# Rudrabha/Wav2Lip

Measured on NVIDIA H100. Metric: 96x96 face-crops/sec (B=128, T=5, mel 80x16), higher is better.
Workload: dtype f16

## Files before the change

wav2lip_b200/csrc/convt_fused.cuh:

```cuda
#pragma once

#include "conv_igemm.cuh"

namespace w2l {

constexpr int kCtThreads = 384;
constexpr int kCtBN = 64;
constexpr int kCtPW = 9, kCtPH = 17;
constexpr int kCtMaxStages = 6;

struct alignas(64) ConvTParams {
    CUtensorMap tmA;
    CUtensorMap tmB;
    CUtensorMap tmO[4];
    int tiles_x, tiles_y, N;
    int kc;
    int stages;
    int patch_bytes, patch_stride;
    int act;
    float cscale[64], cshift[64];
};

template <int G, int BK, bool kBF16>
__device__ __forceinline__ void convt_consumer(const ConvTParams& p, uint32_t smem_base, uint32_t stg, uint32_t bar_base) {
    constexpr int BN = kCtBN;
    constexpr int kRowBytes = BK * 2;
    constexpr int kSlab = BN * BK * 2;
    constexpr uint32_t kSboA = kCtPW * kRowBytes;
    constexpr uint32_t kSboB = 8 * kRowBytes;
    constexpr uint32_t kRowB = BN * 2;
    const int kc = p.kc;
    const int stages = p.stages;
    const uint32_t stage_bytes = p.patch_stride + 9u * kSlab;
    auto full_bar = [&](int s) { return bar_base + 8u * s; };
    auto empty_bar = [&](int s) { return bar_base + 8u * (kCtMaxStages + s); };
    const int lane = threadIdx.x & 31;
    const int q = (threadIdx.x >> 5) & 3;
    const bool leader = (q == 0 && lane == 0);
    const uint32_t bar_id = 1 + G;
    const int tiles_per_img = p.tiles_x * p.tiles_y;
    const int total_units = tiles_per_img * p.N;
    float acc[2][64];
    int stage = 0;
    uint32_t phase = 0;
    for (int unit = blockIdx.x; unit < total_units; unit += gridDim.x) {
        const int n = unit / tiles_per_img;
        const int r = unit - n * tiles_per_img;
        const int ty = r / p.tiles_x, tx = r - ty * p.tiles_x;
        int prev = -1;
        for (int c = 0; c < kc; ++c) {
            mbar_wait(full_bar(stage), phase);
            const uint32_t patch = smem_base + stage * stage_bytes;
            const uint32_t wslab = patch + p.patch_stride;
            wg_fence();
#pragma unroll
            for (int k = 0; k < BK / 16; ++k) {
                const uint32_t on = (c | k) != 0 ? 1u : 0u;
#pragma unroll
                for (int h = 0; h < 2; ++h) {
                    const uint32_t a0 = patch + h * 8 * kSboA + 32u * k;
                    auto ad = [&](uint32_t rows) { return wg_desc(a0 + rows * kRowBytes, 16, kSboA, kRowBytes); };
                    auto bd = [&](int slab) { return wg_desc(wslab + slab * kSlab + 32u * k, 16, kSboB, kRowBytes); };
                    if constexpr (G == 0) {
                        wgmma_m64k16<128, kBF16>(acc[h], ad(0), bd(0), on, 0);
                        wgmma_m64k16<64, kBF16>(acc[h] + 32, ad(1), bd(4), 1u, 0);
                        wgmma_m64k16<64, kBF16>(acc[h] + 32, ad(kCtPW), bd(5), 1u, 0);
                        wgmma_m64k16<64, kBF16>(acc[h] + 32, ad(kCtPW + 1), bd(6), 1u, 0);
                    } else {
                        wgmma_m64k16<128, kBF16>(acc[h], ad(0), bd(2), on, 0);
                        wgmma_m64k16<64, kBF16>(acc[h], ad(1), bd(7), 1u, 0);
                        wgmma_m64k16<64, kBF16>(acc[h] + 32, ad(kCtPW), bd(8), 1u, 0);
                    }
                }
            }
            wg_commit();
            wg_wait<1>();
            if (prev >= 0 && lane == 0) mbar_arrive(empty_bar(prev));
            prev = stage;
            if (++stage == stages) { stage = 0; phase ^= 1u; }
        }
        wg_wait<0>();
        wg_fence_regs<64>(acc[0]);
        wg_fence_regs<64>(acc[1]);
        if (prev >= 0 && lane == 0) mbar_arrive(empty_bar(prev));
#pragma unroll
        for (int lp = 0; lp < 2; ++lp) {
            const int ph = G == 0 ? 3 * lp : 1 + lp;
            if (leader) asm volatile("cp.async.bulk.wait_group.read 0;" ::: "memory");
            named_bar_sync(bar_id, 128);
#pragma unroll
            for (int j = 0; j < 8; ++j) {
                const int cc = 8 * j + 2 * (lane & 3);
                const float sc0 = p.cscale[cc], sc1 = p.cscale[cc + 1], sh0 = p.cshift[cc], sh1 = p.cshift[cc + 1];
#pragma unroll
                for (int h = 0; h < 2; ++h) {
#pragma unroll
                    for (int r8 = 0; r8 < 2; ++r8) {
                        const int row = 64 * h + 16 * q + (lane >> 2) + 8 * r8;
                        float f0 = fmaf(acc[h][4 * (8 * lp + j) + 2 * r8], sc0, sh0);
                        float f1 = fmaf(acc[h][4 * (8 * lp + j) + 2 * r8 + 1], sc1, sh1);
                        if (p.act == ACT_RELU) {
                            f0 = fmaxf(f0, 0.0f);
                            f1 = fmaxf(f1, 0.0f);
                        } else if (p.act == ACT_LRELU) {
                            f0 = f0 > 0.0f ? f0 : 0.01f * f0;
                            f1 = f1 > 0.0f ? f1 : 0.01f * f1;
                        }
                        uint32_t a = stg + row * kRowB + cc * 2;
                        a ^= ((a >> 7) & 7u) << 4;
                        asm volatile("st.shared.b32 [%0], %1;" ::"r"(a), "r"(pack2<kBF16>(f0, f1)) : "memory");
                    }
                }
            }
            asm volatile("fence.proxy.async.shared::cta;" ::: "memory");
            named_bar_sync(bar_id, 128);
            if (leader) {
                asm volatile("cp.async.bulk.tensor.4d.global.shared::cta.bulk_group [%0, {%2, %3, %4, %5}], [%1];"
                             ::"l"(reinterpret_cast<uint64_t>(&p.tmO[ph])), "r"(stg), "r"(0), "r"(tx * 8), "r"(ty * 16), "r"(n)
                             : "memory");
                asm volatile("cp.async.bulk.commit_group;" ::: "memory");
            }
        }
    }
    if (leader) asm volatile("cp.async.bulk.wait_group 0;" ::: "memory");
}

template <int BK, bool kBF16>
__global__ void __launch_bounds__(kCtThreads, 1) convt_fused_kernel(const __grid_constant__ ConvTParams p) {
    pdl_launch_dependents();
    constexpr uint32_t kStgBytes = kTileM * kCtBN * 2;
    constexpr int kSlab = kCtBN * BK * 2;

    extern __shared__ uint8_t smem_raw[];
    const uint32_t smem_base = (smem_u32(smem_raw) + 1023u) & ~1023u;
    const int kc = p.kc;
    const int stages = p.stages;
    const uint32_t stage_bytes = p.patch_stride + 9u * kSlab;
    const uint32_t stg_base = smem_base + stages * stage_bytes;
    const uint32_t bar_base = stg_base + 2u * kStgBytes;
    auto full_bar = [&](int s) { return bar_base + 8u * s; };
    auto empty_bar = [&](int s) { return bar_base + 8u * (kCtMaxStages + s); };

    const int warp = threadIdx.x >> 5;
    const int lane = threadIdx.x & 31;

    if (warp == 0 && lane == 0) {
        tma_prefetch_desc(&p.tmA);
        tma_prefetch_desc(&p.tmB);
#pragma unroll
        for (int i = 0; i < 4; ++i) tma_prefetch_desc(&p.tmO[i]);
    }
    if (warp == 1 && lane == 0) {
        for (int s = 0; s < stages; ++s) {
            mbar_init(full_bar(s), 1);
            mbar_init(empty_bar(s), 8);
        }
        fence_barrier_init();
    }
    __syncthreads();
    pdl_wait();

    const int tiles_per_img = p.tiles_x * p.tiles_y;
    const int total_units = tiles_per_img * p.N;

    if (warp < 4) {
        setmaxnreg_dec<kProducerRegs>();
        if (warp == 0 && lane == 0) {
            int stage = 0;
            uint32_t phase = 0;
            for (int unit = blockIdx.x; unit < total_units; unit += gridDim.x) {
                const int n = unit / tiles_per_img;
                const int r = unit - n * tiles_per_img;
                const int ty = r / p.tiles_x, tx = r - ty * p.tiles_x;
                for (int c = 0; c < kc; ++c) {
                    mbar_wait(empty_bar(stage), phase ^ 1u);
                    const uint32_t a_dst = smem_base + stage * stage_bytes;
                    mbar_arrive_expect_tx(full_bar(stage), static_cast<uint32_t>(p.patch_bytes) + 9u * kSlab);
                    tma_load_4d(a_dst, &p.tmA, full_bar(stage), c * BK, tx * 8, ty * 16, n);
                    tma_load_3d(a_dst + p.patch_stride, &p.tmB, full_bar(stage), c * BK, 0, 0);
                    if (++stage == stages) { stage = 0; phase ^= 1u; }
                }
            }
        }
    } else {
        setmaxnreg_inc<kConsumerRegs>();
        if (warp >= 8)
            convt_consumer<1, BK, kBF16>(p, smem_base, stg_base + kStgBytes, bar_base);
        else
            convt_consumer<0, BK, kBF16>(p, smem_base, stg_base, bar_base);
    }
}

}
```

wav2lip_b200/csrc/host_ops.cuh:

```cuda
#pragma once

static int pick_bk(int cin_pad) { return (cin_pad % 64 == 0) ? 64 : (cin_pad % 32 == 0) ? 32 : 16; }
static int round_up(int a, int b) { return (a + b - 1) / b * b; }
constexpr int kCmMinSteps = 18;
constexpr int kCmMinCtaSteps = 48;
constexpr double kCmFillMargin = 0.06;

static void pick_box(int W, int H, int N, int sx, int sy, int* bw, int* bh, int* bn, int pixels = kTileM) {
    double best = 1e30;
    int b_w = 1, b_h = 1, b_n = 1;
    for (int w = 1; w <= std::min(W, pixels); ++w) {
        if (w * sx > 256) break;
        for (int h = 1; h <= std::min(H, pixels / w); ++h) {
            if (h * sy > 256) break;
            int n = std::min(pixels / (w * h), std::max(N, 1));
            if (n < 1) continue;
            if (n > 256) n = 256;
            const double tiles = (double)((W + w - 1) / w) * ((H + h - 1) / h) * ((N + n - 1) / n);
            const double cost = tiles - 1e-6 * w - 1e-9 * h;
            if (cost < best) { best = cost; b_w = w; b_h = h; b_n = n; }
        }
    }
    *bw = b_w; *bh = b_h; *bn = b_n;
}
// ... 233 lines not shown
    p.bw = bw; p.bh = bh; p.bn = bn;
    p.sx = a.sx; p.sy = a.sy;
    p.ntaps = w.ntaps; p.kc_per_tap = w.cin_pad / BK;
    p.stage_tx_bytes = (unsigned)(op.MT * bw * bh * bn * BK * 2 + BN * BK * 2);
    fill_epi(&p.ep, a);
    p.tma_epi = 0;
    if (ctx->use_tma_epi && !ctx->x2 && !a.head && !a.out.f32) {
        EncodeTiledFn enc = get_encode_fn();
        const int EW = BN < 64 ? BN : 64;
        const CUtensorMapDataType dt = ctx->bf16 ? CU_TENSOR_MAP_DATA_TYPE_BFLOAT16 : CU_TENSOR_MAP_DATA_TYPE_FLOAT16;
        const CUtensorMapSwizzle esw = EW == 64 ? CU_TENSOR_MAP_SWIZZLE_128B : EW == 32 ? CU_TENSOR_MAP_SWIZZLE_64B : CU_TENSOR_MAP_SWIZZLE_32B;
        cuuint64_t dims[4] = {(cuuint64_t)std::min(a.cout, a.out.C), (cuuint64_t)a.Wl, (cuuint64_t)a.Hl, (cuuint64_t)a.in.N};
        cuuint32_t box[4] = {(cuuint32_t)EW, (cuuint32_t)bw, (cuuint32_t)bh, (cuuint32_t)bn};
        cuuint32_t es[4] = {1, 1, 1, 1};
        cuuint64_t os[3] = {(cuuint64_t)p.ep.out_sx * 2, (cuuint64_t)p.ep.out_sy * 2, (cuuint64_t)p.ep.out_sn * 2};
        CUresult r = enc(&p.tmO, dt, 4, p.ep.out, dims, os, box, es, CU_TENSOR_MAP_INTERLEAVE_NONE, esw,
                         CU_TENSOR_MAP_L2_PROMOTION_L2_128B, CU_TENSOR_MAP_FLOAT_OOB_FILL_NONE);
        if (r != CUDA_SUCCESS) return fail(W2L_ECUDA, "%s: cuTensorMapEncodeTiled(out) failed with %d", a.name.c_str(), (int)r);
        if (a.res) {
            cuuint64_t rs[3] = {(cuuint64_t)p.ep.res_sx * 2, (cuuint64_t)p.ep.res_sy * 2, (cuuint64_t)p.ep.res_sn * 2};
            r = enc(&p.tmR, dt, 4, const_cast<void*>(p.ep.res), dims, rs, box, es, CU_TENSOR_MAP_INTERLEAVE_NONE, esw,
                    CU_TENSOR_MAP_L2_PROMOTION_L2_128B, CU_TENSOR_MAP_FLOAT_OOB_FILL_NONE);
            if (r != CUDA_SUCCESS) return fail(W2L_ECUDA, "%s: cuTensorMapEncodeTiled(res) failed with %d", a.name.c_str(), (int)r);
        } else {
            p.tmR = p.tmO;
        }
        p.tma_epi = 1;
        p.epi_box_bytes = (unsigned)(bw * bh * bn * EW * 2);
    }
    if (w.ntaps > kMaxTaps) return fail(W2L_EINVAL, "%s: too many taps", a.name.c_str());
    if (a.cout > a.out.C && !p.tma_epi && !a.head) return fail(W2L_ESTATE, "%s: %d computed channels for a %d-channel destination need the TMA-store epilogue", a.name.c_str(), a.cout, a.out.C);
    if (ctx->x2) {
        if (a.in.lo_off <= 0 || w.nslabs != 2 * w.ntaps) return fail(W2L_ESTATE, "%s: split-operand mode needs hi/lo planes", a.name.c_str());
        int k = 0;
        for (int t = 0; t < w.ntaps; ++t)
            for (int v = 0; v < 3; ++v, ++k) {
                p.dx[k] = w.dx[t]; p.dy[k] = w.dy[t];
                p.a_lo[k] = (v == 1) ? 1 : 0;
                p.b_slab[k] = (unsigned char)((v == 2) ? w.ntaps + t : t);
            }
        p.ntaps = 3 * w.ntaps;
        p.a_lo_off = a.in.lo_off;
    } else {
        for (int t = 0; t < w.ntaps; ++t) { p.dx[t] = w.dx[t]; p.dy[t] = w.dy[t]; p.a_lo[t] = 0; p.b_slab[t] = (unsigned char)t; }
    }
    const int total = ((m_tiles + op.MT - 1) / op.MT) * p.n_tiles;
    op.grid = std::min(total, ctx->num_sms);
    op.fold = w.fold; op.m_tiles = m_tiles; op.n_tiles = p.n_tiles;
    op.flops = 2.0 * a.macs_per_pixel * (double)a.Wl * a.Hl * a.in.N;
    pl->ops.push_back(op);
    return W2L_OK;
}

static int make_convt_fused_op(w2l_ctx* ctx, Plan* pl, const Layer& L, const LayerW& lw, const Act& in, const Act& out, int act = ACT_RELU) {
    EncodeTiledFn enc = get_encode_fn();
    if (!enc) return fail(W2L_ENODEV, "cuTensorMapEncodeTiled is not available");
    const PackedW& w = lw.ph.back();
    Op op;
    op.type = OP_CONV;
    op.name = L.name + " [fused 4-phase]";
    op.ctf = true;
    const int BK = 32;
    if (w.cin_pad % BK != 0) return fail(W2L_EINVAL, "%s: fused convT needs cin %% 32 == 0", L.name.c_str());
    op.BK = BK; op.BN = kCtBN;
    ConvTParams& t = op.tp;
    memset(&t, 0, sizeof(t));
    CKR(encode_act_map(ctx, &t.tmA, in, BK, kCtPW, kCtPH, 1, 1, 1, L.name.c_str()));
    {
        const CUtensorMapDataType dt = ctx->bf16 ? CU_TENSOR_MAP_DATA_TYPE_BFLOAT16 : CU_TENSOR_MAP_DATA_TYPE_FLOAT16;
        const CUtensorMapSwizzle sw = CU_TENSOR_MAP_SWIZZLE_64B;
        cuuint64_t dims[3] = {(cuuint64_t)w.cin_pad, (cuuint64_t)w.cout_pad, 9};
        cuuint64_t strides[2] = {(cuuint64_t)w.cin_pad * 2, (cuuint64_t)w.cin_pad * w.cout_pad * 2};
        cuuint32_t box[3] = {(cuuint32_t)BK, (cuuint32_t)kCtBN, 9};
        cuuint32_t es[3] = {1, 1, 1};
        CUresult r = enc(&t.tmB, dt, 3, w.w, dims, strides, box, es, CU_TENSOR_MAP_INTERLEAVE_NONE, sw,
                         CU_TENSOR_MAP_L2_PROMOTION_L2_256B, CU_TENSOR_MAP_FLOAT_OOB_FILL_NONE);
        if (r != CUDA_SUCCESS) return fail(W2L_ECUDA, "%s: cuTensorMapEncodeTiled(B9) failed with %d", L.name.c_str(), (int)r);
        for (int py = 0; py < 2; ++py)
            for (int px = 0; px < 2; ++px) {
                uint16_t* base = out.base + ((long long)py * out.W + px) * out.Cs + out.c_off;
                cuuint64_t od[4] = {(cuuint64_t)kCtBN, (cuuint64_t)in.W, (cuuint64_t)in.H, (cuuint64_t)in.N};
                cuuint64_t os[3] = {(cuuint64_t)2 * out.Cs * 2, (cuuint64_t)2 * out.W * out.Cs * 2, (cuuint64_t)out.H * out.W * out.Cs * 2};
                cuuint32_t ob[4] = {(cuuint32_t)kCtBN, 8, 16, 1};
                cuuint32_t oe[4] = {1, 1, 1, 1};
                CUresult r2 = enc(&t.tmO[py * 2 + px], dt, 4, base, od, os, ob, oe, CU_TENSOR_MAP_INTERLEAVE_NONE,
                                  CU_TENSOR_MAP_SWIZZLE_128B, CU_TENSOR_MAP_L2_PROMOTION_L2_128B, CU_TENSOR_MAP_FLOAT_OOB_FILL_NONE);
                if (r2 != CUDA_SUCCESS) return fail(W2L_ECUDA, "%s: cuTensorMapEncodeTiled(out phase) failed with %d", L.name.c_str(), (int)r2);
            }
    }
    t.tiles_x = (in.W + 7) / 8; t.tiles_y = (in.H + 15) / 16; t.N = in.N;
    t.kc = w.cin_pad / BK;
    t.patch_bytes = kCtPW * kCtPH * BK * 2;
    t.patch_stride = (t.patch_bytes + 1023) / 1024 * 1024;
    const int stage_bytes = t.patch_stride + 9 * kCtBN * BK * 2;
    const int fixed = 2 * kTileM * kCtBN * 2 + kSmemExtra;
    t.stages = std::min(kCtMaxStages, (kCtSmemMax - fixed) / stage_bytes);
    if (t.stages < 2) return fail(W2L_EINVAL, "%s: fused convT does not fit shared memory", L.name.c_str());
    op.dyn_smem = t.stages * stage_bytes + fixed;
    t.act = act;
    CK(cudaDeviceSynchronize());
    CK(cudaMemcpy(t.cscale, lw.scale, kCtBN * 4, cudaMemcpyDeviceToHost));
    CK(cudaMemcpy(t.cshift, lw.shift, kCtBN * 4, cudaMemcpyDeviceToHost));
    const long long units = (long long)t.tiles_x * t.tiles_y * in.N;
    op.grid = (int)std::min<long long>(units, ctx->num_sms);
    op.m_tiles = (int)units; op.n_tiles = 1;
    op.flops = 2.0 * (double)L.cin * L.cout * 9 * (double)in.W * in.H * in.N;
    pl->ops.push_back(op);
    return W2L_OK;
}

static int emit_block(w2l_ctx* ctx, Plan* pl, const NetW& nw, int li, const Layer& L, const Act& in, const Act& out,
                      const Act* res, bool head = false, int head_B = 1, int head_T = 1, int act_override = -1) {
    const LayerW& lw = nw.layers[li];
    ConvArgs a;
    a.in = in; a.out = out; a.res = res;
    a.scale = lw.scale; a.shift = lw.shift;
    a.act = (L.kind == W2L_BLOCK_CONV_LRELU) ? ACT_LRELU : (L.kind == W2L_BLOCK_CONV_PLAIN ? ACT_NONE : ACT_RELU);
    if (act_override >= 0) a.act = act_override;
    a.cout = L.cout;
    a.head = head; a.head_w = nw.head_w; a.head_b = nw.head_b; a.head_B = head_B; a.head_T = head_T;
    if (L.kind != W2L_BLOCK_CONVT_BN_RELU) {
        a.name = L.name;
        a.w = &lw.ph[0];
        a.sx = lw.ph[0].fold ? 1 : L.sw; a.sy = L.sh;
        a.Hl = out.H; a.Wl = out.W;
        a.macs_per_pixel = (double)L.cin * L.cout * L.kh * L.kw;
        return make_conv_op(ctx, pl, a);
    }
    if (lw.gemm_convT) {
        Act o = out;
        o.H = 1; o.W = 1; o.Cs = out.Cs * out.H * out.W; o.C = L.cout * L.kh * L.kw;
        if (out.c_off != 0 || out.C != out.Cs) return fail(W2L_EINVAL, "%s: gemm convT needs a dense output", L.name.c_str());
        a.name = L.name;
        a.out = o;
        a.w = &lw.ph[0];
        a.Hl = 1; a.Wl = 1;
        a.cout = L.cout * L.kh * L.kw;
        a.macs_per_pixel = (double)L.cin * L.cout * L.kh * L.kw;
        return make_conv_op(ctx, pl, a);
    }
    if (lw.has_all_taps && ctx->use_ctfused && lw.ph.back().cin_pad % 32 == 0 && in.W >= 8 && in.H >= 8 && !res &&
        out.H == 2 * in.H && out.W == 2 * in.W &&
        (double)in.W * in.H / ((double)((in.W + 7) / 8) * ((in.H + 15) / 16) * kTileM) >= 0.6 && !out.f32)
        return make_convt_fused_op(ctx, pl, L, lw, in, out, a.act);
    const size_t nph = lw.ph.size() - (lw.has_all_taps ? 1 : 0);
    for (size_t i = 0; i < nph; ++i) {
        const PackedW& w = lw.ph[i];
        ConvArgs b = a;
        b.name = L.name + ".ph" + std::to_string(w.py) + std::to_string(w.px);
        b.w = &w;
        b.osy = L.sh; b.osx = L.sw; b.phy = w.py; b.phx = w.px;
        b.Hl = (out.H - w.py + L.sh - 1) / L.sh;
        b.Wl = (out.W - w.px + L.sw - 1) / L.sw;
        b.macs_per_pixel = (double)L.cin * L.cout * w.ntaps;
        CKR(make_conv_op(ctx, pl, b));
    }
    return W2L_OK;
}

static void conv_out_dims(const Layer& L, int H, int W, int* Ho, int* Wo) {
    if (L.kind == W2L_BLOCK_CONVT_BN_RELU) {
        *Ho = (H - 1) * L.sh - 2 * L.ph + L.kh + L.out_pad;
        *Wo = (W - 1) * L.sw - 2 * L.pw + L.kw + L.out_pad;
    } else {
        *Ho = (H + 2 * L.ph - L.kh) / L.sh + 1;
        *Wo = (W + 2 * L.pw - L.kw) / L.sw + 1;
    }
}
```

wav2lip_b200/csrc/host_weights.cuh:

```cuda
#pragma once

struct TensorRef { const float* p; int64_t n; };
typedef std::map<std::string, TensorRef> TensorMap;

static int need(const TensorMap& tm, const std::string& name, int64_t numel, const float** out) {
    auto it = tm.find(name);
    if (it == tm.end()) return fail(W2L_EINVAL, "missing tensor '%s'", name.c_str());
    if (it->second.n != numel) return fail(W2L_EINVAL, "tensor '%s' has %lld elements, expected %lld", name.c_str(), (long long)it->second.n, (long long)numel);
    *out = it->second.p;
    return W2L_OK;
}

static int pack_taps(w2l_ctx* ctx, LayerW* lw, PackedW* pw, const float* src, int cout, int cin, int kh, int kw, bool transposed,
                     const std::vector<std::pair<int, int>>& rs, int cout_pad_to, RepackLog* log, cudaStream_t st,
                     uint16_t* dst_override = nullptr) {
    PackParams pp;
    memset(&pp, 0, sizeof(pp));
    pp.src = src;
    pp.ntaps = (int)rs.size();
    pp.cout = cout; pp.cin = cin;
    pp.cin_pad = round_up(cin, 16);
    pp.cout_pad = round_up(cout, cout_pad_to);
    if (transposed) { pp.s_ci = (long long)cout * kh * kw; pp.s_co = (long long)kh * kw; }
    else { pp.s_co = (long long)cin * kh * kw; pp.s_ci = (long long)kh * kw; }
// ... 40 lines not shown
        CKR(alloc_in(ctx, &lw->mem, &pw.w, n * 2));
        PackFoldParams fp;
        fp.src = W; fp.dst = pw.w; fp.kh = L.kh; fp.kw = L.kw; fp.cout = L.cout; fp.cin = L.cin;
        fp.cout_pad = pw.cout_pad; fp.kfold = pw.kfold; fp.Cp = pw.Cp;
        const int blocks = (int)std::min<size_t>((n + 255) / 256, 4096);
        if (log) log->pack_fold.push_back(fp);
        if (ctx->bf16) pack_fold_kernel<true><<<blocks, 256, 0, st>>>(fp);
        else pack_fold_kernel<false><<<blocks, 256, 0, st>>>(fp);
        ctx->launches++;
        CK(cudaGetLastError());
        lw->ph.push_back(pw);
    } else if (L.kind != W2L_BLOCK_CONVT_BN_RELU) {
        std::vector<std::pair<int, int>> rs;
        PackedW pw;
        for (int r = 0; r < L.kh; ++r)
            for (int s = 0; s < L.kw; ++s) { rs.push_back({r, s}); pw.dy.push_back((signed char)(r - L.ph)); pw.dx.push_back((signed char)(s - L.pw)); }
        CKR(pack_taps(ctx, lw, &pw, W, L.cout_real > 0 ? L.cout_real : L.cout, L.cin, L.kh, L.kw, false, rs, pad_to, log, st));
        lw->ph.push_back(pw);
    } else if (in_hw1 && !ctx->x2 && L.sh == 1 && L.sw == 1 && L.ph == 0 && L.pw == 0) {
        lw->gemm_convT = true;
        reps = L.kh * L.kw;
        PackedW pw;
        pw.ntaps = 1; pw.cin_pad = round_up(L.cin, 16); pw.cout_pad = round_up(L.cout, pad_to) * reps;
        pw.dx.push_back(0); pw.dy.push_back(0);
        CKR(alloc_in(ctx, &lw->mem, &pw.w, (size_t)pw.cout_pad * pw.cin_pad * 2));
        if (L.cout % pad_to != 0) return fail(W2L_EINVAL, "%s: gemm convT needs cout %% 16 == 0", L.name.c_str());
        for (int r = 0; r < L.kh; ++r)
            for (int s = 0; s < L.kw; ++s) {
                std::vector<std::pair<int, int>> rs = {{r, s}};
                CKR(pack_taps(ctx, lw, nullptr, W, L.cout, L.cin, L.kh, L.kw, true, rs, pad_to, log, st,
                              pw.w + (size_t)(r * L.kw + s) * L.cout * pw.cin_pad));
            }
        lw->ph.push_back(pw);
    } else {
        for (int py = 0; py < L.sh; ++py)
            for (int px = 0; px < L.sw; ++px) {
                std::vector<std::pair<int, int>> rs;
                PackedW pw;
                pw.py = py; pw.px = px;
                for (int r = 0; r < L.kh; ++r) {
                    if ((py + L.ph - r) % L.sh != 0) continue;
                    for (int s = 0; s < L.kw; ++s) {
                        if ((px + L.pw - s) % L.sw != 0) continue;
                        rs.push_back({r, s});
                        pw.dy.push_back((signed char)((py + L.ph - r) / L.sh));
                        pw.dx.push_back((signed char)((px + L.pw - s) / L.sw));
                    }
                }
                if (rs.empty()) return fail(W2L_EINVAL, "%s: empty transposed-conv phase", L.name.c_str());
                CKR(pack_taps(ctx, lw, &pw, W, L.cout, L.cin, L.kh, L.kw, true, rs, pad_to, log, st));
                lw->ph.push_back(pw);
            }
        if (!ctx->x2 && L.cout == kCtBN && L.kh == 3 && L.kw == 3 && L.sh == 2 && L.sw == 2 && L.ph == 1 && L.pw == 1 && L.out_pad == 1) {
            std::vector<std::pair<int, int>> rs = {{1, 1}, {2, 2}, {1, 2}, {2, 1},
                                                   {2, 0}, {0, 2}, {0, 0},
                                                   {1, 0},
                                                   {0, 1}};
            PackedW pw;
            for (int t = 0; t < 9; ++t) { pw.dy.push_back(0); pw.dx.push_back(0); }
            CKR(pack_taps(ctx, lw, &pw, W, L.cout, L.cin, L.kh, L.kw, true, rs, pad_to, log, st));
            lw->ph.push_back(pw);
            lw->has_all_taps = true;
        }
    }
    const int n_pad = round_up(L.cout, pad_to) * reps;
    CKR(alloc_in(ctx, &lw->mem, &lw->scale, (size_t)n_pad * 4));
    CKR(alloc_in(ctx, &lw->mem, &lw->shift, (size_t)n_pad * 4));
    lw->n_scale = n_pad;
    fold_bn_kernel<<<(n_pad + 127) / 128, 128, 0, st>>>(bias, gamma, beta, mean, var, 1e-5f, L.cout_real > 0 ? L.cout_real : L.cout, reps, n_pad, lw->scale, lw->shift);
    if (log && bias) log->fold.push_back(FoldJob{bias, L.cout, reps, n_pad, lw->scale, lw->shift});
    ctx->launches++;
    CK(cudaGetLastError());
    lw->loaded = true;
    return W2L_OK;
}

static int fetch_block_tensors(const TensorMap& tm, const Layer& L, const float** W, const float** b, const float** g,
                               const float** be, const float** m, const float** v) {
    const int cout = L.cout_real > 0 ? L.cout_real : L.cout;
    const int64_t wn = (int64_t)L.cin * cout * L.kh * L.kw;
    CKR(need(tm, L.name + (L.bare_keys ? ".weight" : ".conv_block.0.weight"), wn, W));
    CKR(need(tm, L.name + (L.bare_keys ? ".bias" : ".conv_block.0.bias"), cout, b));
    *g = *be = *m = *v = nullptr;
    if (L.kind == W2L_BLOCK_CONV_BN_RELU || L.kind == W2L_BLOCK_CONVT_BN_RELU) {
        CKR(need(tm, L.name + ".conv_block.1.weight", L.cout, g));
        CKR(need(tm, L.name + ".conv_block.1.bias", L.cout, be));
        CKR(need(tm, L.name + ".conv_block.1.running_mean", L.cout, m));
        CKR(need(tm, L.name + ".conv_block.1.running_var", L.cout, v));
    }
    return W2L_OK;
}

static void drop_plans(w2l_ctx* ctx, int net) {
    for (auto it = ctx->plans.begin(); it != ctx->plans.end();) {
        if (it->second->net == net) it = ctx->plans.erase(it);
        else ++it;
    }
    ctx->last_plan[net] = nullptr;
    ctx->plan_epoch[net]++;
}
```

wav2lip_b200/csrc/conv_igemm.cuh:

```cuda
#pragma once

#include <cuda.h>
#include <cuda_bf16.h>
#include <cuda_fp16.h>
#include <stdint.h>

#include "wgmma.cuh"

namespace w2l {

constexpr int kTileM = 128;
constexpr int kMaxTaps = 49;
constexpr int kMaxSteps = 3 * kMaxTaps;
constexpr int kSmemExtra = 2048;
constexpr int kSmemMax = 227 * 1024;

enum : int { ACT_NONE = 0, ACT_RELU = 1, ACT_LRELU = 2 };

struct EpiParams {
    int Wout, Hout, N;
    int act;
    int out_f32;
    void* out;
    long long out_sn, out_sy, out_sx;
// ... 85 lines not shown
__device__ __forceinline__ void wg_mma_tile(float (&acc)[2][BN / 2], uint32_t a, uint32_t sbo_a, uint32_t b, bool accumulate) {
#pragma unroll
    for (int k = 0; k < BK / 16; ++k) {
        const uint64_t bd = make_kmajor_desc<BK>(b + 32u * k);
        const uint32_t on = (accumulate || k > 0) ? 1u : 0u;
        wgmma_m64k16<BN, kBF16>(acc[0], wg_desc(a + 32u * k, 16, sbo_a, BK * 2), bd, on, 0);
        wgmma_m64k16<BN, kBF16>(acc[1], wg_desc(a + 8u * sbo_a + 32u * k, 16, sbo_a, BK * 2), bd, on, 0);
    }
}

constexpr int kCmPixels = 256;
template <int BN, int BK, int MT = 1, bool kCM = false>
struct ConvCfg {
    static constexpr int kRowsA = kCM ? kCmPixels : kTileM;
    static constexpr int kATile = kRowsA * BK * 2;
    static constexpr int kABytes = MT * kATile;
    static constexpr int kBBytes = BN * BK * 2;
    static constexpr int kStageBytes = kABytes + kBBytes;
    static constexpr int kEW = BN < 64 ? BN : 64;
    static constexpr int kCW = BN < 32 ? BN : 32;
    static constexpr int kPasses = kCM ? 1 : BN / kEW;
    static constexpr int kBoxBytes = kRowsA * kEW * 2;
    static constexpr int kGrpRaw = (kCM || kPasses * kBoxBytes > xbuf_bytes<kCW>()) ? kPasses * kBoxBytes : xbuf_bytes<kCW>();
    static constexpr int kGrpBytes = (kGrpRaw + 1023) / 1024 * 1024;
    static constexpr int kStagesRaw = (kSmemMax - kSmemExtra - 2 * kGrpBytes) / kStageBytes;
    static constexpr int kStages = kStagesRaw > 8 ? 8 : kStagesRaw;
    static constexpr int kRingBytes = (kStages * kStageBytes + 1023) / 1024 * 1024;
    static constexpr int kSmemBytes = kRingBytes + 2 * kGrpBytes + kSmemExtra;
    static constexpr int kThreads = 384;
    static_assert(BN <= 128, "a warpgroup holds at most 128 fp32 accumulator columns per row");
    static_assert(!kCM || (BN == 128 && BK == 64 && MT == 1), "channel-major form: 128 channels, 128-byte K rows, one tile");
    static_assert(kBoxBytes % 1024 == 0, "staging boxes must keep the 1024-byte swizzle alignment");
    static_assert(kStages >= 2, "need a pipeline");
    static_assert(kSmemBytes <= kSmemMax, "shared-memory carve-up exceeds the per-CTA limit");
};

__device__ int g_f16_overflow = 0;

template <bool kBF16>
__device__ __forceinline__ uint32_t pack2_live(float a, float b, uint32_t live_bits) {
    if constexpr (kBF16) {
        __nv_bfloat162 h = __floats2bfloat162_rn(a, b);
        return *reinterpret_cast<uint32_t*>(&h);
    } else {
        __half2 h = __floats2half2_rn(a, b);
        const uint32_t u = *reinterpret_cast<uint32_t*>(&h);
        if (((u & 0x7FFF7FFFu) + 0x04000400u) & live_bits) g_f16_overflow = 1;
        return u;
    }
}
template <bool kBF16>
__device__ __forceinline__ uint32_t pack2(float a, float b, bool live = true) {
    return pack2_live<kBF16>(a, b, live ? 0x80008000u : 0u);
}
template <bool kBF16>
__device__ __forceinline__ float2 unpack2(uint32_t u) {
    if constexpr (kBF16) {
        return __bfloat1622float2(*reinterpret_cast<__nv_bfloat162*>(&u));
    } else {
        return __half22float2(*reinterpret_cast<__half2*>(&u));
    }
}

template <int BN, bool kBF16, bool kHead>
__device__ __forceinline__ void epilogue_tile(const EpiParams& e, const float (&acc)[2][BN / 2], float* xb, uint32_t bar_id,
                                              bool valid, int n, int y, int x, int nt) {
    constexpr int CH = (BN >= 32) ? 32 : 16;
    const long long o_off = (long long)n * e.out_sn + (long long)y * e.out_sy + (long long)x * e.out_sx;
    const long long r_off = (long long)n * e.res_sn + (long long)y * e.res_sy + (long long)x * e.res_sx;
#pragma unroll
    for (int c0 = 0; c0 < BN; c0 += CH) {
        uint32_t v[CH];
        acc_to_rows<CH>(acc[0], acc[1], c0, xb, bar_id, v);
        if (valid) {
            const int cg = nt * BN + c0;
            float f[CH];
#pragma unroll
            for (int j = 0; j < CH; j += 4) {
                const float4 sc = __ldg(reinterpret_cast<const float4*>(e.scale + cg + j));
                const float4 sh = __ldg(reinterpret_cast<const float4*>(e.shift + cg + j));
                f[j + 0] = fmaf(__uint_as_float(v[j + 0]), sc.x, sh.x);
                f[j + 1] = fmaf(__uint_as_float(v[j + 1]), sc.y, sh.y);
                f[j + 2] = fmaf(__uint_as_float(v[j + 2]), sc.z, sh.z);
                f[j + 3] = fmaf(__uint_as_float(v[j + 3]), sc.w, sh.w);
            }
            if (e.res != nullptr) {
                const uint4* rp = reinterpret_cast<const uint4*>(
                    reinterpret_cast<const uint16_t*>(e.res) + r_off + cg);
#pragma unroll
                for (int j = 0; j < CH / 8; ++j) {
                    const uint4 r = __ldg(rp + j);
                    const float2 a = unpack2<kBF16>(r.x), b = unpack2<kBF16>(r.y);
                    const float2 c = unpack2<kBF16>(r.z), d = unpack2<kBF16>(r.w);
                    f[8 * j + 0] += a.x; f[8 * j + 1] += a.y; f[8 * j + 2] += b.x; f[8 * j + 3] += b.y;
                    f[8 * j + 4] += c.x; f[8 * j + 5] += c.y; f[8 * j + 6] += d.x; f[8 * j + 7] += d.y;
                }
                if (e.x2) {
#pragma unroll
                    for (int j = 0; j < CH / 8; ++j) {
                        const uint4 r = __ldg(rp + (e.res_lo_off >> 3) + j);
                        const float2 a = unpack2<kBF16>(r.x), b = unpack2<kBF16>(r.y);
                        const float2 c = unpack2<kBF16>(r.z), d = unpack2<kBF16>(r.w);
                        f[8 * j + 0] += a.x; f[8 * j + 1] += a.y; f[8 * j + 2] += b.x; f[8 * j + 3] += b.y;
                        f[8 * j + 4] += c.x; f[8 * j + 5] += c.y; f[8 * j + 6] += d.x; f[8 * j + 7] += d.y;
                    }
                }
// ... 436 lines not shown
```

Baseline: 60780.

## Split fused convT output channels across CTA pairs with resident weights

Each CTA pair now splits the 64 output channels into two halves of 32. Each CTA loads its half of the weights once into shared memory, so the ring only streams activation patches, which allows deeper stages. The two consumer warpgroups alternate whole units through named-barrier handoff instead of splitting phases, the taps are reordered to suit the new wgmma grouping, and the epilogue double-buffers the staging tiles. The cost is that each CTA pair loads every activation patch twice, and the layers that fit shared memory are now limited by the resident weights.

```diff
diff --git a/wav2lip_b200/csrc/convt_fused.cuh b/wav2lip_b200/csrc/convt_fused.cuh
--- a/wav2lip_b200/csrc/convt_fused.cuh
+++ b/wav2lip_b200/csrc/convt_fused.cuh
@@ -6,8 +6,16 @@
 
 constexpr int kCtThreads = 384;
 constexpr int kCtBN = 64;
+constexpr int kCtHalf = 32;
 constexpr int kCtPW = 9, kCtPH = 17;
-constexpr int kCtMaxStages = 6;
+constexpr int kCtMaxStages = 12;
+constexpr int kCtStgBytes = kTileM * kCtHalf * 2;
+constexpr int kCtStgPerGroup = 2;
+constexpr int kCtBK = 32;
+constexpr int kCtPatchStride = (kCtPW * kCtPH * kCtBK * 2 + 1023) / 1024 * 1024;
+constexpr int convt_fused_fixed_smem(int cin_pad) {
+    return 9 * kCtHalf * cin_pad * 2 + 2 * kCtStgPerGroup * kCtStgBytes + kSmemExtra;
+}
 
 struct alignas(64) ConvTParams {
     CUtensorMap tmA;
@@ -22,36 +30,44 @@
 };
 
 template <int G, int BK, bool kBF16>
-__device__ __forceinline__ void convt_consumer(const ConvTParams& p, uint32_t smem_base, uint32_t stg, uint32_t bar_base) {
-    constexpr int BN = kCtBN;
+__device__ __forceinline__ void convt_consumer(const ConvTParams& p, uint32_t wts, uint32_t ring, uint32_t stg,
+                                               uint32_t bar_base) {
     constexpr int kRowBytes = BK * 2;
-    constexpr int kSlab = BN * BK * 2;
+    constexpr int kWChunk = 9 * kCtHalf * kRowBytes;
     constexpr uint32_t kSboA = kCtPW * kRowBytes;
     constexpr uint32_t kSboB = 8 * kRowBytes;
-    constexpr uint32_t kRowB = BN * 2;
+    constexpr uint32_t kSlab = kCtHalf * kRowBytes;
+    constexpr uint32_t kRowB = kCtHalf * 2;
     const int kc = p.kc;
     const int stages = p.stages;
-    const uint32_t stage_bytes = p.patch_stride + 9u * kSlab;
     auto full_bar = [&](int s) { return bar_base + 8u * s; };
     auto empty_bar = [&](int s) { return bar_base + 8u * (kCtMaxStages + s); };
+    const uint32_t w_bar = bar_base + 8u * (2 * kCtMaxStages);
     const int lane = threadIdx.x & 31;
     const int q = (threadIdx.x >> 5) & 3;
     const bool leader = (q == 0 && lane == 0);
     const uint32_t bar_id = 1 + G;
+    constexpr uint32_t my_turn = 3 + G, their_turn = 3 + (G ^ 1);
+    const int half = blockIdx.x & 1;
+    const int pair = blockIdx.x >> 1, pairs = gridDim.x >> 1;
     const int tiles_per_img = p.tiles_x * p.tiles_y;
     const int total_units = tiles_per_img * p.N;
+    const float* const cscale = p.cscale + kCtHalf * half;
+    const float* const cshift = p.cshift + kCtHalf * half;
+    mbar_wait(w_bar, 0);
     float acc[2][64];
-    int stage = 0;
-    uint32_t phase = 0;
-    for (int unit = blockIdx.x; unit < total_units; unit += gridDim.x) {
-        const int n = unit / tiles_per_img;
-        const int r = unit - n * tiles_per_img;
-        const int ty = r / p.tiles_x, tx = r - ty * p.tiles_x;
+    for (int i = G;; i += 2) {
+        const int unit = pair + i * pairs;
+        if (unit >= total_units) break;
+        if (i > 0) named_bar_sync(my_turn, 256);
+        const int s0 = i * kc;
+        int stage = s0 % stages;
+        uint32_t phase = static_cast<uint32_t>(s0 / stages) & 1u;
         int prev = -1;
         for (int c = 0; c < kc; ++c) {
             mbar_wait(full_bar(stage), phase);
-            const uint32_t patch = smem_base + stage * stage_bytes;
-            const uint32_t wslab = patch + p.patch_stride;
+            const uint32_t patch = ring + stage * p.patch_stride;
+            const uint32_t wc = wts + c * kWChunk;
             wg_fence();
 #pragma unroll
             for (int k = 0; k < BK / 16; ++k) {
@@ -60,17 +76,13 @@
                 for (int h = 0; h < 2; ++h) {
                     const uint32_t a0 = patch + h * 8 * kSboA + 32u * k;
                     auto ad = [&](uint32_t rows) { return wg_desc(a0 + rows * kRowBytes, 16, kSboA, kRowBytes); };
-                    auto bd = [&](int slab) { return wg_desc(wslab + slab * kSlab + 32u * k, 16, kSboB, kRowBytes); };
-                    if constexpr (G == 0) {
-                        wgmma_m64k16<128, kBF16>(acc[h], ad(0), bd(0), on, 0);
-                        wgmma_m64k16<64, kBF16>(acc[h] + 32, ad(1), bd(4), 1u, 0);
-                        wgmma_m64k16<64, kBF16>(acc[h] + 32, ad(kCtPW), bd(5), 1u, 0);
-                        wgmma_m64k16<64, kBF16>(acc[h] + 32, ad(kCtPW + 1), bd(6), 1u, 0);
-                    } else {
-                        wgmma_m64k16<128, kBF16>(acc[h], ad(0), bd(2), on, 0);
-                        wgmma_m64k16<64, kBF16>(acc[h], ad(1), bd(7), 1u, 0);
-                        wgmma_m64k16<64, kBF16>(acc[h] + 32, ad(kCtPW), bd(8), 1u, 0);
-                    }
+                    auto bd = [&](int slab) { return wg_desc(wc + slab * kSlab + 32u * k, 16, kSboB, kRowBytes); };
+                    wgmma_m64k16<64, kBF16>(acc[h], ad(0), bd(0), on, 0);
+                    wgmma_m64k16<64, kBF16>(acc[h] + 32, ad(0), bd(2), on, 0);
+                    wgmma_m64k16<64, kBF16>(acc[h], ad(1), bd(4), 1u, 0);
+                    wgmma_m64k16<32, kBF16>(acc[h], ad(kCtPW), bd(6), 1u, 0);
+                    wgmma_m64k16<32, kBF16>(acc[h] + 32, ad(kCtPW), bd(7), 1u, 0);
+                    wgmma_m64k16<32, kBF16>(acc[h], ad(kCtPW + 1), bd(8), 1u, 0);
                 }
             }
             wg_commit();
@@ -79,26 +91,31 @@
             prev = stage;
             if (++stage == stages) { stage = 0; phase ^= 1u; }
         }
+        if (pair + (i + 1) * pairs < total_units) named_bar_arrive(their_turn, 256);
         wg_wait<0>();
         wg_fence_regs<64>(acc[0]);
         wg_fence_regs<64>(acc[1]);
-        if (prev >= 0 && lane == 0) mbar_arrive(empty_bar(prev));
-#pragma unroll
-        for (int lp = 0; lp < 2; ++lp) {
-            const int ph = G == 0 ? 3 * lp : 1 + lp;
-            if (leader) asm volatile("cp.async.bulk.wait_group.read 0;" ::: "memory");
+        if (lane == 0) mbar_arrive(empty_bar(prev));
+        const int n = unit / tiles_per_img;
+        const int r = unit - n * tiles_per_img;
+        const int ty = r / p.tiles_x, tx = r - ty * p.tiles_x;
+#pragma unroll
+        for (int lp = 0; lp < 4; ++lp) {
+            const int ph = (0x0213 >> (4 * lp)) & 15;
+            const uint32_t tile = stg + (lp & 1) * kCtStgBytes;
+            if (leader) asm volatile("cp.async.bulk.wait_group.read 1;" ::: "memory");
             named_bar_sync(bar_id, 128);
 #pragma unroll
-            for (int j = 0; j < 8; ++j) {
+            for (int j = 0; j < 4; ++j) {
                 const int cc = 8 * j + 2 * (lane & 3);
-                const float sc0 = p.cscale[cc], sc1 = p.cscale[cc + 1], sh0 = p.cshift[cc], sh1 = p.cshift[cc + 1];
+                const float sc0 = cscale[cc], sc1 = cscale[cc + 1], sh0 = cshift[cc], sh1 = cshift[cc + 1];
 #pragma unroll
                 for (int h = 0; h < 2; ++h) {
 #pragma unroll
                     for (int r8 = 0; r8 < 2; ++r8) {
                         const int row = 64 * h + 16 * q + (lane >> 2) + 8 * r8;
-                        float f0 = fmaf(acc[h][4 * (8 * lp + j) + 2 * r8], sc0, sh0);
-                        float f1 = fmaf(acc[h][4 * (8 * lp + j) + 2 * r8 + 1], sc1, sh1);
+                        float f0 = fmaf(acc[h][4 * (4 * lp + j) + 2 * r8], sc0, sh0);
+                        float f1 = fmaf(acc[h][4 * (4 * lp + j) + 2 * r8 + 1], sc1, sh1);
                         if (p.act == ACT_RELU) {
                             f0 = fmaxf(f0, 0.0f);
                             f1 = fmaxf(f1, 0.0f);
@@ -106,8 +123,8 @@
                             f0 = f0 > 0.0f ? f0 : 0.01f * f0;
                             f1 = f1 > 0.0f ? f1 : 0.01f * f1;
                         }
-                        uint32_t a = stg + row * kRowB + cc * 2;
-                        a ^= ((a >> 7) & 7u) << 4;
+                        uint32_t a = tile + row * kRowB + cc * 2;
+                        a ^= ((a >> 7) & 3u) << 4;
                         asm volatile("st.shared.b32 [%0], %1;" ::"r"(a), "r"(pack2<kBF16>(f0, f1)) : "memory");
                     }
                 }
@@ -116,7 +133,8 @@
             named_bar_sync(bar_id, 128);
             if (leader) {
                 asm volatile("cp.async.bulk.tensor.4d.global.shared::cta.bulk_group [%0, {%2, %3, %4, %5}], [%1];"
-                             ::"l"(reinterpret_cast<uint64_t>(&p.tmO[ph])), "r"(stg), "r"(0), "r"(tx * 8), "r"(ty * 16), "r"(n)
+                             ::"l"(reinterpret_cast<uint64_t>(&p.tmO[ph])), "r"(tile), "r"(kCtHalf * half), "r"(tx * 8),
+                               "r"(ty * 16), "r"(n)
                              : "memory");
                 asm volatile("cp.async.bulk.commit_group;" ::: "memory");
             }
@@ -128,18 +146,20 @@
 template <int BK, bool kBF16>
 __global__ void __launch_bounds__(kCtThreads, 1) convt_fused_kernel(const __grid_constant__ ConvTParams p) {
     pdl_launch_dependents();
-    constexpr uint32_t kStgBytes = kTileM * kCtBN * 2;
-    constexpr int kSlab = kCtBN * BK * 2;
+    constexpr uint32_t kWChunk = 9 * kCtHalf * BK * 2;
+    constexpr uint32_t kGrpStg = kCtStgPerGroup * kCtStgBytes;
 
     extern __shared__ uint8_t smem_raw[];
     const uint32_t smem_base = (smem_u32(smem_raw) + 1023u) & ~1023u;
     const int kc = p.kc;
     const int stages = p.stages;
-    const uint32_t stage_bytes = p.patch_stride + 9u * kSlab;
-    const uint32_t stg_base = smem_base + stages * stage_bytes;
-    const uint32_t bar_base = stg_base + 2u * kStgBytes;
+    const uint32_t wts = smem_base;
+    const uint32_t ring = wts + kc * kWChunk;
+    const uint32_t stg_base = ring + stages * p.patch_stride;
+    const uint32_t bar_base = stg_base + 2u * kGrpStg;
     auto full_bar = [&](int s) { return bar_base + 8u * s; };
     auto empty_bar = [&](int s) { return bar_base + 8u * (kCtMaxStages + s); };
+    const uint32_t w_bar = bar_base + 8u * (2 * kCtMaxStages);
 
     const int warp = threadIdx.x >> 5;
     const int lane = threadIdx.x & 31;
@@ -153,8 +173,9 @@
     if (warp == 1 && lane == 0) {
         for (int s = 0; s < stages; ++s) {
             mbar_init(full_bar(s), 1);
-            mbar_init(empty_bar(s), 8);
-        }
+            mbar_init(empty_bar(s), 4);
+        }
+        mbar_init(w_bar, 1);
         fence_barrier_init();
     }
     __syncthreads();
@@ -162,22 +183,24 @@
 
     const int tiles_per_img = p.tiles_x * p.tiles_y;
     const int total_units = tiles_per_img * p.N;
+    const int half = blockIdx.x & 1;
+    const int pair = blockIdx.x >> 1, pairs = gridDim.x >> 1;
 
     if (warp < 4) {
         setmaxnreg_dec<kProducerRegs>();
         if (warp == 0 && lane == 0) {
+            mbar_arrive_expect_tx(w_bar, static_cast<uint32_t>(kc) * kWChunk);
+            for (int c = 0; c < kc; ++c) tma_load_3d(wts + c * kWChunk, &p.tmB, w_bar, c * BK, kCtHalf * half, 0);
             int stage = 0;
             uint32_t phase = 0;
-            for (int unit = blockIdx.x; unit < total_units; unit += gridDim.x) {
+            for (int unit = pair; unit < total_units; unit += pairs) {
                 const int n = unit / tiles_per_img;
                 const int r = unit - n * tiles_per_img;
                 const int ty = r / p.tiles_x, tx = r - ty * p.tiles_x;
                 for (int c = 0; c < kc; ++c) {
                     mbar_wait(empty_bar(stage), phase ^ 1u);
-                    const uint32_t a_dst = smem_base + stage * stage_bytes;
-                    mbar_arrive_expect_tx(full_bar(stage), static_cast<uint32_t>(p.patch_bytes) + 9u * kSlab);
-                    tma_load_4d(a_dst, &p.tmA, full_bar(stage), c * BK, tx * 8, ty * 16, n);
-                    tma_load_3d(a_dst + p.patch_stride, &p.tmB, full_bar(stage), c * BK, 0, 0);
+                    mbar_arrive_expect_tx(full_bar(stage), static_cast<uint32_t>(p.patch_bytes));
+                    tma_load_4d(ring + stage * p.patch_stride, &p.tmA, full_bar(stage), c * BK, tx * 8, ty * 16, n);
                     if (++stage == stages) { stage = 0; phase ^= 1u; }
                 }
             }
@@ -185,10 +208,10 @@
     } else {
         setmaxnreg_inc<kConsumerRegs>();
         if (warp >= 8)
-            convt_consumer<1, BK, kBF16>(p, smem_base, stg_base + kStgBytes, bar_base);
+            convt_consumer<1, BK, kBF16>(p, wts, ring, stg_base + kGrpStg, bar_base);
         else
-            convt_consumer<0, BK, kBF16>(p, smem_base, stg_base, bar_base);
-    }
-}
-
-}
+            convt_consumer<0, BK, kBF16>(p, wts, ring, stg_base, bar_base);
+    }
+}
+
+}
diff --git a/wav2lip_b200/csrc/host_ops.cuh b/wav2lip_b200/csrc/host_ops.cuh
--- a/wav2lip_b200/csrc/host_ops.cuh
+++ b/wav2lip_b200/csrc/host_ops.cuh
@@ -309,6 +309,10 @@
     return W2L_OK;
 }
 
+static bool convt_fused_fits(int cin_pad) {
+    return cin_pad % kCtBK == 0 && convt_fused_fixed_smem(cin_pad) + 4 * kCtPatchStride <= kCtSmemMax;
+}
+
 static int make_convt_fused_op(w2l_ctx* ctx, Plan* pl, const Layer& L, const LayerW& lw, const Act& in, const Act& out, int act = ACT_RELU) {
     EncodeTiledFn enc = get_encode_fn();
     if (!enc) return fail(W2L_ENODEV, "cuTensorMapEncodeTiled is not available");
@@ -317,8 +321,8 @@
     op.type = OP_CONV;
     op.name = L.name + " [fused 4-phase]";
     op.ctf = true;
-    const int BK = 32;
-    if (w.cin_pad % BK != 0) return fail(W2L_EINVAL, "%s: fused convT needs cin %% 32 == 0", L.name.c_str());
+    const int BK = kCtBK;
+    if (!convt_fused_fits(w.cin_pad)) return fail(W2L_EINVAL, "%s: fused convT does not fit shared memory", L.name.c_str());
     op.BK = BK; op.BN = kCtBN;
     ConvTParams& t = op.tp;
     memset(&t, 0, sizeof(t));
@@ -328,7 +332,7 @@
         const CUtensorMapSwizzle sw = CU_TENSOR_MAP_SWIZZLE_64B;
         cuuint64_t dims[3] = {(cuuint64_t)w.cin_pad, (cuuint64_t)w.cout_pad, 9};
         cuuint64_t strides[2] = {(cuuint64_t)w.cin_pad * 2, (cuuint64_t)w.cin_pad * w.cout_pad * 2};
-        cuuint32_t box[3] = {(cuuint32_t)BK, (cuuint32_t)kCtBN, 9};
+        cuuint32_t box[3] = {(cuuint32_t)BK, (cuuint32_t)kCtHalf, 9};
         cuuint32_t es[3] = {1, 1, 1};
         CUresult r = enc(&t.tmB, dt, 3, w.w, dims, strides, box, es, CU_TENSOR_MAP_INTERLEAVE_NONE, sw,
                          CU_TENSOR_MAP_L2_PROMOTION_L2_256B, CU_TENSOR_MAP_FLOAT_OOB_FILL_NONE);
@@ -338,28 +342,26 @@
                 uint16_t* base = out.base + ((long long)py * out.W + px) * out.Cs + out.c_off;
                 cuuint64_t od[4] = {(cuuint64_t)kCtBN, (cuuint64_t)in.W, (cuuint64_t)in.H, (cuuint64_t)in.N};
                 cuuint64_t os[3] = {(cuuint64_t)2 * out.Cs * 2, (cuuint64_t)2 * out.W * out.Cs * 2, (cuuint64_t)out.H * out.W * out.Cs * 2};
-                cuuint32_t ob[4] = {(cuuint32_t)kCtBN, 8, 16, 1};
+                cuuint32_t ob[4] = {(cuuint32_t)kCtHalf, 8, 16, 1};
                 cuuint32_t oe[4] = {1, 1, 1, 1};
                 CUresult r2 = enc(&t.tmO[py * 2 + px], dt, 4, base, od, os, ob, oe, CU_TENSOR_MAP_INTERLEAVE_NONE,
-                                  CU_TENSOR_MAP_SWIZZLE_128B, CU_TENSOR_MAP_L2_PROMOTION_L2_128B, CU_TENSOR_MAP_FLOAT_OOB_FILL_NONE);
+                                  CU_TENSOR_MAP_SWIZZLE_64B, CU_TENSOR_MAP_L2_PROMOTION_L2_128B, CU_TENSOR_MAP_FLOAT_OOB_FILL_NONE);
                 if (r2 != CUDA_SUCCESS) return fail(W2L_ECUDA, "%s: cuTensorMapEncodeTiled(out phase) failed with %d", L.name.c_str(), (int)r2);
             }
     }
     t.tiles_x = (in.W + 7) / 8; t.tiles_y = (in.H + 15) / 16; t.N = in.N;
     t.kc = w.cin_pad / BK;
     t.patch_bytes = kCtPW * kCtPH * BK * 2;
-    t.patch_stride = (t.patch_bytes + 1023) / 1024 * 1024;
-    const int stage_bytes = t.patch_stride + 9 * kCtBN * BK * 2;
-    const int fixed = 2 * kTileM * kCtBN * 2 + kSmemExtra;
-    t.stages = std::min(kCtMaxStages, (kCtSmemMax - fixed) / stage_bytes);
-    if (t.stages < 2) return fail(W2L_EINVAL, "%s: fused convT does not fit shared memory", L.name.c_str());
-    op.dyn_smem = t.stages * stage_bytes + fixed;
+    t.patch_stride = kCtPatchStride;
+    const int fixed = convt_fused_fixed_smem(w.cin_pad);
+    t.stages = std::min(kCtMaxStages, (kCtSmemMax - fixed) / t.patch_stride);
+    op.dyn_smem = t.stages * t.patch_stride + fixed;
     t.act = act;
     CK(cudaDeviceSynchronize());
     CK(cudaMemcpy(t.cscale, lw.scale, kCtBN * 4, cudaMemcpyDeviceToHost));
     CK(cudaMemcpy(t.cshift, lw.shift, kCtBN * 4, cudaMemcpyDeviceToHost));
     const long long units = (long long)t.tiles_x * t.tiles_y * in.N;
-    op.grid = (int)std::min<long long>(units, ctx->num_sms);
+    op.grid = (int)std::min<long long>(2 * units, ctx->num_sms & ~1);
     op.m_tiles = (int)units; op.n_tiles = 1;
     op.flops = 2.0 * (double)L.cin * L.cout * 9 * (double)in.W * in.H * in.N;
     pl->ops.push_back(op);
@@ -396,7 +398,7 @@
         a.macs_per_pixel = (double)L.cin * L.cout * L.kh * L.kw;
         return make_conv_op(ctx, pl, a);
     }
-    if (lw.has_all_taps && ctx->use_ctfused && lw.ph.back().cin_pad % 32 == 0 && in.W >= 8 && in.H >= 8 && !res &&
+    if (lw.has_all_taps && ctx->use_ctfused && convt_fused_fits(lw.ph.back().cin_pad) && in.W >= 8 && in.H >= 8 && !res &&
         out.H == 2 * in.H && out.W == 2 * in.W &&
         (double)in.W * in.H / ((double)((in.W + 7) / 8) * ((in.H + 15) / 16) * kTileM) >= 0.6 && !out.f32)
         return make_convt_fused_op(ctx, pl, L, lw, in, out, a.act);
diff --git a/wav2lip_b200/csrc/host_weights.cuh b/wav2lip_b200/csrc/host_weights.cuh
--- a/wav2lip_b200/csrc/host_weights.cuh
+++ b/wav2lip_b200/csrc/host_weights.cuh
@@ -116,10 +116,10 @@
                 lw->ph.push_back(pw);
             }
         if (!ctx->x2 && L.cout == kCtBN && L.kh == 3 && L.kw == 3 && L.sh == 2 && L.sw == 2 && L.ph == 1 && L.pw == 1 && L.out_pad == 1) {
-            std::vector<std::pair<int, int>> rs = {{1, 1}, {2, 2}, {1, 2}, {2, 1},
-                                                   {2, 0}, {0, 2}, {0, 0},
-                                                   {1, 0},
-                                                   {0, 1}};
+            std::vector<std::pair<int, int>> rs = {{2, 2}, {1, 2}, {2, 1}, {1, 1},
+                                                   {2, 0}, {1, 0},
+                                                   {0, 2}, {0, 1},
+                                                   {0, 0}};
             PackedW pw;
             for (int t = 0; t < 9; ++t) { pw.dy.push_back(0); pw.dx.push_back(0); }
             CKR(pack_taps(ctx, lw, &pw, W, L.cout, L.cin, L.kh, L.kw, true, rs, pad_to, log, st));
```

Result: faster. 61510 (median of 6 runs) (+1.2%).

## Double-buffer convT epilogue staging and specialize activation at compile time

Applied to the files above, without the earlier changes.

Gives each consumer warpgroup two staging tiles in the fused transposed-conv epilogue, so it waits only for the older bulk store (wait_group.read 1) instead of draining every TMA store before writing the next phase. The activation branch becomes a compile-time template via integral_constant, and the f16 overflow check is OR-accumulated and flagged once per tile rather than per pack. The extra staging memory can reduce the number of pipeline stages that fit in shared memory.

```diff
diff --git a/wav2lip_b200/csrc/conv_igemm.cuh b/wav2lip_b200/csrc/conv_igemm.cuh
--- a/wav2lip_b200/csrc/conv_igemm.cuh
+++ b/wav2lip_b200/csrc/conv_igemm.cuh
@@ -161,6 +161,21 @@
 template <bool kBF16>
 __device__ __forceinline__ uint32_t pack2(float a, float b, bool live = true) {
     return pack2_live<kBF16>(a, b, live ? 0x80008000u : 0u);
+}
+template <bool kBF16>
+__device__ __forceinline__ uint32_t pack2_ovf(float a, float b, uint32_t& ovf) {
+    if constexpr (kBF16) {
+        return pack2_live<true>(a, b, 0u);
+    } else {
+        __half2 h = __floats2half2_rn(a, b);
+        const uint32_t u = *reinterpret_cast<uint32_t*>(&h);
+        ovf |= (u & 0x7FFF7FFFu) + 0x04000400u;
+        return u;
+    }
+}
+template <bool kBF16>
+__device__ __forceinline__ void f16_flag_set(uint32_t ovf) {
+    if (!kBF16 && (ovf & 0x80008000u)) g_f16_overflow = 1;
 }
 template <bool kBF16>
 __device__ __forceinline__ float2 unpack2(uint32_t u) {
diff --git a/wav2lip_b200/csrc/convt_fused.cuh b/wav2lip_b200/csrc/convt_fused.cuh
--- a/wav2lip_b200/csrc/convt_fused.cuh
+++ b/wav2lip_b200/csrc/convt_fused.cuh
@@ -1,4 +1,6 @@
 #pragma once
+
+#include <type_traits>
 
 #include "conv_igemm.cuh"
 
@@ -8,6 +10,7 @@
 constexpr int kCtBN = 64;
 constexpr int kCtPW = 9, kCtPH = 17;
 constexpr int kCtMaxStages = 6;
+constexpr uint32_t kCtStgBytes = kTileM * kCtBN * 2;
 
 struct alignas(64) ConvTParams {
     CUtensorMap tmA;
@@ -83,44 +86,53 @@
         wg_fence_regs<64>(acc[0]);
         wg_fence_regs<64>(acc[1]);
         if (prev >= 0 && lane == 0) mbar_arrive(empty_bar(prev));
-#pragma unroll
-        for (int lp = 0; lp < 2; ++lp) {
-            const int ph = G == 0 ? 3 * lp : 1 + lp;
-            if (leader) asm volatile("cp.async.bulk.wait_group.read 0;" ::: "memory");
-            named_bar_sync(bar_id, 128);
-#pragma unroll
-            for (int j = 0; j < 8; ++j) {
-                const int cc = 8 * j + 2 * (lane & 3);
-                const float sc0 = p.cscale[cc], sc1 = p.cscale[cc + 1], sh0 = p.cshift[cc], sh1 = p.cshift[cc + 1];
-#pragma unroll
-                for (int h = 0; h < 2; ++h) {
-#pragma unroll
-                    for (int r8 = 0; r8 < 2; ++r8) {
-                        const int row = 64 * h + 16 * q + (lane >> 2) + 8 * r8;
-                        float f0 = fmaf(acc[h][4 * (8 * lp + j) + 2 * r8], sc0, sh0);
-                        float f1 = fmaf(acc[h][4 * (8 * lp + j) + 2 * r8 + 1], sc1, sh1);
-                        if (p.act == ACT_RELU) {
-                            f0 = fmaxf(f0, 0.0f);
-                            f1 = fmaxf(f1, 0.0f);
-                        } else if (p.act == ACT_LRELU) {
-                            f0 = f0 > 0.0f ? f0 : 0.01f * f0;
-                            f1 = f1 > 0.0f ? f1 : 0.01f * f1;
+        auto epilogue = [&](auto act_c) {
+            constexpr int kAct = decltype(act_c)::value;
+            uint32_t ovf = 0;
+#pragma unroll
+            for (int lp = 0; lp < 2; ++lp) {
+                const int ph = G == 0 ? 3 * lp : 1 + lp;
+                const uint32_t tile = stg + lp * kCtStgBytes;
+                if (leader) asm volatile("cp.async.bulk.wait_group.read 1;" ::: "memory");
+                named_bar_sync(bar_id, 128);
+#pragma unroll
+                for (int j = 0; j < 8; ++j) {
+                    const int cc = 8 * j + 2 * (lane & 3);
+                    const float sc0 = p.cscale[cc], sc1 = p.cscale[cc + 1], sh0 = p.cshift[cc], sh1 = p.cshift[cc + 1];
+#pragma unroll
+                    for (int h = 0; h < 2; ++h) {
+#pragma unroll
+                        for (int r8 = 0; r8 < 2; ++r8) {
+                            const int row = 64 * h + 16 * q + (lane >> 2) + 8 * r8;
+                            float f0 = fmaf(acc[h][4 * (8 * lp + j) + 2 * r8], sc0, sh0);
+                            float f1 = fmaf(acc[h][4 * (8 * lp + j) + 2 * r8 + 1], sc1, sh1);
+                            if constexpr (kAct == ACT_RELU) {
+                                f0 = fmaxf(f0, 0.0f);
+                                f1 = fmaxf(f1, 0.0f);
+                            } else if constexpr (kAct == ACT_LRELU) {
+                                f0 = f0 > 0.0f ? f0 : 0.01f * f0;
+                                f1 = f1 > 0.0f ? f1 : 0.01f * f1;
+                            }
+                            uint32_t o = row * kRowB + cc * 2;
+                            o ^= ((o >> 7) & 7u) << 4;
+                            asm volatile("st.shared.b32 [%0], %1;" ::"r"(tile + o), "r"(pack2_ovf<kBF16>(f0, f1, ovf)) : "memory");
                         }
-                        uint32_t a = stg + row * kRowB + cc * 2;
-                        a ^= ((a >> 7) & 7u) << 4;
-                        asm volatile("st.shared.b32 [%0], %1;" ::"r"(a), "r"(pack2<kBF16>(f0, f1)) : "memory");
                     }
                 }
+                asm volatile("fence.proxy.async.shared::cta;" ::: "memory");
+                named_bar_sync(bar_id, 128);
+                if (leader) {
+                    asm volatile("cp.async.bulk.tensor.4d.global.shared::cta.bulk_group [%0, {%2, %3, %4, %5}], [%1];"
+                                 ::"l"(reinterpret_cast<uint64_t>(&p.tmO[ph])), "r"(tile), "r"(0), "r"(tx * 8), "r"(ty * 16), "r"(n)
+                                 : "memory");
+                    asm volatile("cp.async.bulk.commit_group;" ::: "memory");
+                }
             }
-            asm volatile("fence.proxy.async.shared::cta;" ::: "memory");
-            named_bar_sync(bar_id, 128);
-            if (leader) {
-                asm volatile("cp.async.bulk.tensor.4d.global.shared::cta.bulk_group [%0, {%2, %3, %4, %5}], [%1];"
-                             ::"l"(reinterpret_cast<uint64_t>(&p.tmO[ph])), "r"(stg), "r"(0), "r"(tx * 8), "r"(ty * 16), "r"(n)
-                             : "memory");
-                asm volatile("cp.async.bulk.commit_group;" ::: "memory");
-            }
-        }
+            f16_flag_set<kBF16>(ovf);
+        };
+        if (p.act == ACT_RELU) epilogue(std::integral_constant<int, ACT_RELU>{});
+        else if (p.act == ACT_LRELU) epilogue(std::integral_constant<int, ACT_LRELU>{});
+        else epilogue(std::integral_constant<int, ACT_NONE>{});
     }
     if (leader) asm volatile("cp.async.bulk.wait_group 0;" ::: "memory");
 }
@@ -128,7 +140,7 @@
 template <int BK, bool kBF16>
 __global__ void __launch_bounds__(kCtThreads, 1) convt_fused_kernel(const __grid_constant__ ConvTParams p) {
     pdl_launch_dependents();
-    constexpr uint32_t kStgBytes = kTileM * kCtBN * 2;
+    constexpr uint32_t kStgBytes = 2 * kCtStgBytes;
     constexpr int kSlab = kCtBN * BK * 2;
 
     extern __shared__ uint8_t smem_raw[];
diff --git a/wav2lip_b200/csrc/host_ops.cuh b/wav2lip_b200/csrc/host_ops.cuh
--- a/wav2lip_b200/csrc/host_ops.cuh
+++ b/wav2lip_b200/csrc/host_ops.cuh
@@ -350,7 +350,7 @@
     t.patch_bytes = kCtPW * kCtPH * BK * 2;
     t.patch_stride = (t.patch_bytes + 1023) / 1024 * 1024;
     const int stage_bytes = t.patch_stride + 9 * kCtBN * BK * 2;
-    const int fixed = 2 * kTileM * kCtBN * 2 + kSmemExtra;
+    const int fixed = 4 * (int)kCtStgBytes + kSmemExtra;
     t.stages = std::min(kCtMaxStages, (kCtSmemMax - fixed) / stage_bytes);
     if (t.stages < 2) return fail(W2L_EINVAL, "%s: fused convT does not fit shared memory", L.name.c_str());
     op.dyn_smem = t.stages * stage_bytes + fixed;
```

Result: faster. 61160 before, 62380 after (median of 6 runs) (+2.0%).
